# snap-research/R2L

Hardware: AMD Instinct MI355X
Metric: rays/sec (train+render) W256D88 lego@400x400 (higher is better)
Workload: dtype f32 (v_mfma_f32_32x32x2_f32: exact fp32 products and accumulate)

## Files before the change

### r2l_amd/csrc/r2l_dw.h

```cpp
#pragma once
#include "r2l_student_net.h"

#define DW_CHUNK 64
#ifndef DW_DEPTH
#define DW_DEPTH 4
#endif
#ifndef DW_LONG_TRIP
#define DW_LONG_TRIP 128
#endif

struct R2LDwArgs {
    const float* save_x;
    const float* save_t;
    const float* gx;
    const float* gt;
    float* grads;
    int n_block;
    int layer0;
    int n_layers;
    int64_t N;
    int64_t units_per_layer;
    int64_t units_per_wg;
    float* slab;
    float unscale = 1.0f;
    const float* scale_dev = nullptr;
    unsigned* status = nullptr;
    const unsigned* run_if = nullptr;
    unsigned mid_off = 0u;
    const float* act_scale = nullptr;
};

#define DW_SLAB_FLOATS (R2L_W * R2L_W + R2L_W)
#define DW_MAX_WGS 256
#define DW_HEAD_SLAB_MAX ((int64_t)64 * R2L_W * 1024)
#define DW_BODY_SLAB ((int64_t)DW_MAX_WGS * 2 * DW_SLAB_FLOATS)
#define DW_TAIL_SLAB_BASE (DW_BODY_SLAB + DW_HEAD_SLAB_MAX)
#define DW_TAIL_SLAB ((int64_t)512 * 4 * R2L_W)

struct R2LDwHeadArgs {
    const float* rays_o;
    const float* rays_d;
    const float* t_rand;
    const float* ztab;
    const float* emb;
    const float* gh;
    float* slab;
    float* grads;
    int64_t N;
    int64_t rays_per_wg;
    float gscale = 1.0f, unscale = 1.0f;
    const float* scale_dev = nullptr;
    const unsigned* run_unless = nullptr;
    const unsigned* run_if = nullptr;
    bool exact = false;
};

struct PECol {
    int smp, ax;
    float scale;
    int kind;
};
__device__ __forceinline__ PECol pe_col(int k) {
    PECol c;
    if (k >= R2L_IN) { c.smp = 0; c.ax = 0; c.scale = 0.f; c.kind = 3; return c; }
    const int co = k / 21, f = k - 21 * co;
    c.smp = co / 3;
    c.ax = co - 3 * c.smp;
    c.kind = f == 20 ? 2 : (f < 10 ? 0 : 1);
    c.scale = f == 20 ? 1.f : (float)(1 << (f < 10 ? f : f - 10));
    return c;
}
__device__ __forceinline__ float pe_eval(const PECol& c, float x) {
    float s, co;
    r2l_sincos(x * c.scale, s, co);
    const float t = c.kind == 0 ? s : co;
    return c.kind == 2 ? x : (c.kind == 3 ? 0.f : t);
}

int r2l_dw_head16_launch(const R2LDwHeadArgs& a, int64_t slices, hipStream_t stream);

int r2l_dw16_launch(const R2LDwArgs& a, int64_t wgs, const unsigned* run_unless, hipStream_t stream);

int r2l_bwd2_open_step(unsigned* status, const float* params, int n_block, float grad_scale, const float* drgb, int64_t N,
                       hipStream_t stream);
int r2l_dw_body_launch(R2LDwArgs a, int dw_body, int64_t wgs, unsigned* status, bool no_fallback, hipStream_t stream);
int r2l_dw_head_launch(R2LDwHeadArgs a, int64_t slices, bool dw_head16, const unsigned* status, bool no_fallback,
                       hipStream_t stream);
int r2l_dw_tail_launch(const float* dpre, const float* x0, const float* xn, float* grads, float* part, int n_block, int64_t N,
                       int64_t wgs, int64_t rays_per_wg, hipStream_t stream);
```

### r2l_amd/csrc/r2l_dw_head.hip

```cpp
#include "r2l_dw.h"

struct HeadStep {
    f32x4 g0, g1;
    float o0, d0, u0, o1, d1, u1;
};

template <bool FROM_EMB, bool JITTER>
__global__ __launch_bounds__(256, 1) void r2l_dw_head_kernel(const R2LDwHeadArgs a) {
    if (a.run_if != nullptr && __builtin_nontemporal_load(a.run_if) == 0u) return;
    const int wave = threadIdx.x >> 6, lane = threadIdx.x & 63;
    const int hh = lane >> 5, jl = lane & 31;
    const int kq = blockIdx.x & 3;
    const int64_t slice = blockIdx.x >> 2;
    const int64_t r0 = slice * a.rays_per_wg;
    int64_t r1 = r0 + a.rays_per_wg;
    if (r1 > a.N) r1 = a.N;
    if (r0 >= r1) return;
    const int kbase = kq * 256 + wave * 64;
    constexpr bool from_emb = FROM_EMB;
    constexpr bool jitter = JITTER && !FROM_EMB;
    const int k0 = kbase + jl, k1 = kbase + 32 + jl;
    const PECol c0 = pe_col(k0), c1 = pe_col(k1);
    const int e0 = k0 < R2L_IN ? k0 : R2L_IN - 1, e1 = k1 < R2L_IN ? k1 : R2L_IN - 1;
    const float m0 = k0 < R2L_IN ? 1.f : 0.f, m1 = k1 < R2L_IN ? 1.f : 0.f;
    const float zl0 = from_emb ? 0.f : a.ztab[c0.smp], zs0 = jitter ? a.ztab[16 + c0.smp] : 0.f;
    const float zl1 = from_emb ? 0.f : a.ztab[c1.smp], zs1 = jitter ? a.ztab[16 + c1.smp] : 0.f;

    f32x16 acc[8][2];
#pragma unroll
    for (int eo = 0; eo < 8; ++eo)
#pragma unroll
        for (int ei = 0; ei < 2; ++ei)
#pragma unroll
            for (int c = 0; c < 16; ++c) acc[eo][ei][c] = 0.f;
    f32x4 bs0 = {0.f, 0.f, 0.f, 0.f}, bs1 = {0.f, 0.f, 0.f, 0.f};

    const int64_t nfull = (r1 - r0) / 2;
    auto ld = [&](int64_t s, HeadStep& v) {
        const int64_t sc = s < nfull ? s : (nfull > 0 ? nfull - 1 : 0);
        const int64_t r = r0 + 2 * sc + hh;
        v.g0 = *reinterpret_cast<const f32x4*>(a.gh + r * R2L_W + 4 * jl);
        v.g1 = *reinterpret_cast<const f32x4*>(a.gh + r * R2L_W + 128 + 4 * jl);
        if constexpr (from_emb) {
            v.o0 = a.emb[r * R2L_IN + e0];
            v.o1 = a.emb[r * R2L_IN + e1];
            v.d0 = v.d1 = v.u0 = v.u1 = 0.f;
        } else {
            v.o0 = a.rays_o[r * 3 + c0.ax]; v.d0 = a.rays_d[r * 3 + c0.ax];
            v.o1 = a.rays_o[r * 3 + c1.ax]; v.d1 = a.rays_d[r * 3 + c1.ax];
            if constexpr (jitter) {
                v.u0 = a.t_rand[r * 16 + c0.smp];
                v.u1 = a.t_rand[r * 16 + c1.smp];
            } else {
                v.u0 = v.u1 = 0.f;
            }
        }
    };
    auto encode = [&](const HeadStep& v, float& p0, float& p1) {
        if constexpr (from_emb) { p0 = v.o0 * m0; p1 = v.o1 * m1; return; }
        const float z0 = jitter ? zl0 + zs0 * v.u0 : zl0;
        const float z1 = jitter ? zl1 + zs1 * v.u1 : zl1;
        p0 = pe_eval(c0, v.o0 + v.d0 * z0);
        p1 = pe_eval(c1, v.o1 + v.d1 * z1);
    };
    auto kstep = [&](const f32x4& g0, const f32x4& g1, float p0, float p1) {
#pragma unroll
        for (int e = 0; e < 4; ++e) {
            acc[e][0] = __builtin_amdgcn_mfma_f32_32x32x2f32(g0[e], p0, acc[e][0], 0, 0, 0);
            acc[e][1] = __builtin_amdgcn_mfma_f32_32x32x2f32(g0[e], p1, acc[e][1], 0, 0, 0);
            acc[4 + e][0] = __builtin_amdgcn_mfma_f32_32x32x2f32(g1[e], p0, acc[4 + e][0], 0, 0, 0);
            acc[4 + e][1] = __builtin_amdgcn_mfma_f32_32x32x2f32(g1[e], p1, acc[4 + e][1], 0, 0, 0);
        }
        bs0 += g0;
        bs1 += g1;
    };
    if (nfull > 0) {
        HeadStep hb[4];
#pragma unroll
        for (int k = 0; k < 4; ++k) ld(k, hb[k]);
        float pa0, pa1;
        encode(hb[0], pa0, pa1);
        int64_t s = 0;
        for (; s + 16 <= nfull; s += 16) {
#pragma unroll
            for (int k = 0; k < 16; ++k) {
                const f32x4 g0 = hb[k & 3].g0, g1 = hb[k & 3].g1;
                float pn0, pn1;
                encode(hb[(k + 1) & 3], pn0, pn1);
                kstep(g0, g1, pa0, pa1);
                ld(s + k + 4, hb[k & 3]);
                pa0 = pn0;
                pa1 = pn1;
                __builtin_amdgcn_sched_barrier(0);
            }
        }
        for (; s < nfull; ++s) {
            HeadStep v;
            ld(s, v);
            float p0, p1;
            encode(v, p0, p1);
            kstep(v.g0, v.g1, p0, p1);
        }
    }
    if ((r1 - r0) & 1) {
        const int64_t r = r1 - 1;
        HeadStep v;
        v.g0 = *reinterpret_cast<const f32x4*>(a.gh + r * R2L_W + 4 * jl);
        v.g1 = *reinterpret_cast<const f32x4*>(a.gh + r * R2L_W + 128 + 4 * jl);
        if constexpr (from_emb) {
            v.o0 = a.emb[r * R2L_IN + e0];
            v.o1 = a.emb[r * R2L_IN + e1];
            v.d0 = v.d1 = v.u0 = v.u1 = 0.f;
        } else {
            v.o0 = a.rays_o[r * 3 + c0.ax]; v.d0 = a.rays_d[r * 3 + c0.ax];
            v.o1 = a.rays_o[r * 3 + c1.ax]; v.d1 = a.rays_d[r * 3 + c1.ax];
            v.u0 = jitter ? a.t_rand[r * 16 + c0.smp] : 0.f;
            v.u1 = jitter ? a.t_rand[r * 16 + c1.smp] : 0.f;
        }
        float p0, p1;
        encode(v, p0, p1);
        if (hh) { v.g0 = f32x4{0.f, 0.f, 0.f, 0.f}; v.g1 = v.g0; p0 = 0.f; p1 = 0.f; }
        kstep(v.g0, v.g1, p0, p1);
    }
    float* gw = a.grads;
    float* sl = a.slab ? a.slab + slice * (int64_t)(R2L_W * 1024) : nullptr;
#pragma unroll
    for (int eo = 0; eo < 8; ++eo)
#pragma unroll
        for (int ei = 0; ei < 2; ++ei)
#pragma unroll
            for (int c = 0; c < 16; ++c) {
                const int ro = (c & 3) + 8 * (c >> 2) + 4 * hh;
                const int o = (eo >> 2) * 128 + 4 * ro + (eo & 3);
                const int k = kbase + ei * 32 + jl;
                if (k < R2L_IN) {
                    if (sl) sl[o * 1024 + k] = acc[eo][ei][c];
                    else atomicAdd(gw + (int64_t)o * R2L_IN + k, acc[eo][ei][c]);
                }
            }
    if (kq == 0 && wave == 0) {
        float* gb = a.grads + r2l_off_head_b();
#pragma unroll
        for (int e = 0; e < 4; ++e) {
            const float s0 = bs0[e] + __shfl_xor(bs0[e], 32);
            const float s1 = bs1[e] + __shfl_xor(bs1[e], 32);
            if (hh == 0) {
                if (sl) {
                    sl[(4 * jl + e) * 1024 + R2L_IN] = s0;
                    sl[(128 + 4 * jl + e) * 1024 + R2L_IN] = s1;
                } else {
                    atomicAdd(gb + 4 * jl + e, s0);
                    atomicAdd(gb + 128 + 4 * jl + e, s1);
                }
            }
        }
    }
}

__global__ void r2l_head_reduce_kernel(const float* __restrict__ slab, int n_slices, float* __restrict__ grads) {
    const int64_t i = (int64_t)blockIdx.x * blockDim.x + threadIdx.x;
    if (i >= (int64_t)R2L_W * 1024) return;
    const int o = (int)(i >> 10), k = (int)(i & 1023);
    if (k > R2L_IN) return;
    float s = 0.f;
    for (int sidx = 0; sidx < n_slices; ++sidx) s += slab[(int64_t)sidx * (R2L_W * 1024) + i];
    if (k == R2L_IN) grads[r2l_off_head_b() + o] += s;
    else grads[(int64_t)o * R2L_IN + k] += s;
}

int r2l_dw_head_launch(R2LDwHeadArgs a, int64_t slices, bool dw_head16, const unsigned* status, bool no_fallback,
                       hipStream_t stream) {
    const dim3 hg((unsigned)(slices * 4)), hb(256);
    if (dw_head16) {
        a.run_unless = status;
        if (const int rc = r2l_dw_head16_launch(a, slices, stream)) return rc;
        a.run_unless = nullptr;
        a.run_if = status;
    }
    if (dw_head16 && no_fallback) {
    } else if (a.emb != nullptr) hipLaunchKernelGGL((r2l_dw_head_kernel<true, false>), hg, hb, 0, stream, a);
    else if (a.t_rand != nullptr) hipLaunchKernelGGL((r2l_dw_head_kernel<false, true>), hg, hb, 0, stream, a);
    else hipLaunchKernelGGL((r2l_dw_head_kernel<false, false>), hg, hb, 0, stream, a);
    R2L_CHECK(hipGetLastError());
    if (a.slab) {
        hipLaunchKernelGGL(r2l_head_reduce_kernel, dim3(R2L_W * 1024 / 256), dim3(256), 0, stream, a.slab, (int)slices, a.grads);
        R2L_CHECK(hipGetLastError());
    }
    return 0;
}
```

### r2l_amd/csrc/r2l_dw_head16.hip

```cpp
#include "r2l_f2.h"
#include "r2l_dw.h"

struct Head16G {
    float g[8][8];
};
struct Head16Rays {
    float oa[8], da[8], ua[8], ob[8], db[8], ub[8];
};
struct Head16Pair {
    int ka, kb;
    int smp_a, ax_a;
    int smp_b, ax_b;
    float scale;
    bool trig;
};
__device__ __forceinline__ Head16Pair head16_pair(int P) {
    Head16Pair c;
    if (P < 480) {
        const int co = P / 10, f = P - 10 * co;
        c.ka = 21 * co + f; c.kb = 21 * co + 10 + f;
        c.smp_a = c.smp_b = co / 3; c.ax_a = c.ax_b = co % 3;
        c.scale = (float)(1 << f); c.trig = true;
    } else {
        const int i = P - 480, ca = 2 * i, cb = 2 * i + 1;
        const bool live = i < 24;
        c.ka = live ? 21 * ca + 20 : -1; c.kb = live ? 21 * cb + 20 : -1;
        c.smp_a = live ? ca / 3 : 0; c.ax_a = live ? ca % 3 : 0;
        c.smp_b = live ? cb / 3 : 0; c.ax_b = live ? cb % 3 : 0;
        c.scale = 1.f; c.trig = false;
    }
    return c;
}

typedef __amdgpu_buffer_rsrc_t h16_rsrc_t;
__device__ __forceinline__ float h16_load(h16_rsrc_t rs, unsigned voff, unsigned imm) {
    return __builtin_bit_cast(float, __builtin_amdgcn_raw_buffer_load_b32(rs, voff + imm, 0, 0));
}
__device__ __forceinline__ h16_rsrc_t h16_rsrc(const float* base, unsigned bytes) {
    return __builtin_amdgcn_make_buffer_rsrc(const_cast<float*>(base), 0, (int)bytes, 0x00020000);
}

template <bool JITTER, bool EXACT>
__global__ __launch_bounds__(256, 1) void r2l_dw_head16_kernel(const R2LDwHeadArgs a) {
    if (a.run_unless != nullptr && __builtin_nontemporal_load(a.run_unless) != 0u) return;
    const float gscale = a.scale_dev != nullptr ? a.scale_dev[0] : a.gscale;
    const float unscale = a.scale_dev != nullptr ? a.scale_dev[1] : a.unscale;
    const int lane = threadIdx.x & 63;
    const int wave = __builtin_amdgcn_readfirstlane((int)(threadIdx.x >> 6));
    const int m = lane & 31, kg = lane >> 5;
    const int kq = blockIdx.x & 3;
    const int64_t slice = blockIdx.x >> 2;
    const int64_t r0 = slice * a.rays_per_wg;
    int64_t r1 = r0 + a.rays_per_wg;
    if (r1 > a.N) r1 = a.N;
    if (r0 >= r1) return;
    const int nrays = (int)(r1 - r0);
    const Head16Pair pc = head16_pair(kq * 128 + wave * 32 + m);
    const bool trig_wave = kq * 128 + wave * 32 + 31 < 480;
    const float zla = a.ztab[pc.smp_a], zsa = JITTER ? a.ztab[16 + pc.smp_a] : 0.f;
    const float zlb = a.ztab[pc.smp_b], zsb = JITTER ? a.ztab[16 + pc.smp_b] : 0.f;

    f32x16 acc[8][2];
#pragma unroll
    for (int e = 0; e < 8; ++e)
#pragma unroll
        for (int ei = 0; ei < 2; ++ei)
#pragma unroll
            for (int c = 0; c < 16; ++c) acc[e][ei][c] = 0.f;
    float bsum[8] = {0.f, 0.f, 0.f, 0.f, 0.f, 0.f, 0.f, 0.f};

    const h16_rsrc_t grs = h16_rsrc(a.gh + r0 * R2L_W, (unsigned)nrays * (R2L_W * 4));
    const h16_rsrc_t ors = h16_rsrc(a.rays_o + r0 * 3, (unsigned)nrays * 12u);
    const h16_rsrc_t drs = h16_rsrc(a.rays_d + r0 * 3, (unsigned)nrays * 12u);
    const h16_rsrc_t urs = h16_rsrc(JITTER ? a.t_rand + r0 * 16 : a.rays_o, JITTER ? (unsigned)nrays * 64u : 0u);
    unsigned vg = (unsigned)((8 * kg * R2L_W + m) * 4);
    unsigned vp0 = (unsigned)((8 * kg * 3 + pc.ax_a) * 4), vp1 = (unsigned)((8 * kg * 3 + pc.ax_b) * 4);
    unsigned vu0 = (unsigned)((8 * kg * 16 + pc.smp_a) * 4), vu1 = (unsigned)((8 * kg * 16 + pc.smp_b) * 4);
    const int nsteps = (nrays + 15) / 16;

    auto ld_g = [&](Head16G& v) {
#pragma unroll
        for (int i = 0; i < 8; ++i)
#pragma unroll
            for (int e = 0; e < 8; ++e)
                v.g[e][i] = (i < 4) ? h16_load(grs, vg, (unsigned)(i * 1024 + e * 128))
                                    : h16_load(grs, vg + 4096u, (unsigned)((i - 4) * 1024 + e * 128));
        vg += 16u * R2L_W * 4u;
    };
    auto ld_rays = [&](Head16Rays& v) {
#pragma unroll
        for (int i = 0; i < 8; ++i) {
            v.oa[i] = h16_load(ors, vp0, (unsigned)i * 12u);
            v.da[i] = h16_load(drs, vp0, (unsigned)i * 12u);
            v.ua[i] = JITTER ? h16_load(urs, vu0, (unsigned)i * 64u) : 0.f;
            if (!trig_wave) {
                v.ob[i] = h16_load(ors, vp1, (unsigned)i * 12u);
                v.db[i] = h16_load(drs, vp1, (unsigned)i * 12u);
                v.ub[i] = JITTER ? h16_load(urs, vu1, (unsigned)i * 64u) : 0.f;
            } else {
                v.ob[i] = v.db[i] = v.ub[i] = 0.f;
            }
        }
        vp0 += 16u * 12u; vp1 += 16u * 12u;
        vu0 += 16u * 64u; vu1 += 16u * 64u;
    };
    auto pk = [](float x0, float x1) { return F2Side<false, F3None>::pk(x0, x1); };
    Head16G rg;
    Head16Rays rr;
    ld_g(rg);
    ld_rays(rr);
    for (int s = 0; s < nsteps; ++s) {
        f16x8 ga[8], gm[EXACT ? 8 : 1];
        const float sc = gscale;
#pragma unroll
        for (int e = 0; e < 8; ++e) {
            u32x4 uh;
#pragma unroll
            for (int d = 0; d < 4; ++d) uh[d] = pk(rg.g[e][2 * d] * sc, rg.g[e][2 * d + 1] * sc);
            ga[e] = __builtin_bit_cast(f16x8, uh);
            if (EXACT) {
                u32x4 um;
#pragma unroll
                for (int d = 0; d < 4; ++d)
                    um[d] = pk(f2_res_lo(uh[d], rg.g[e][2 * d] * sc), f2_res_hi(uh[d], rg.g[e][2 * d + 1] * sc));
                gm[e] = __builtin_bit_cast(f16x8, um);
            }
            if (kq == 0 && wave == 0)
                bsum[e] += ((rg.g[e][0] + rg.g[e][1]) + (rg.g[e][2] + rg.g[e][3])) + ((rg.g[e][4] + rg.g[e][5]) + (rg.g[e][6] + rg.g[e][7]));
        }
        __builtin_amdgcn_sched_barrier(0);
        ld_g(rg);
        __builtin_amdgcn_sched_barrier(0);
        float p0[8], p1[8];
#pragma unroll
        for (int i = 0; i < 8; ++i) {
            const float xa = rr.oa[i] + rr.da[i] * (JITTER ? zla + zsa * rr.ua[i] : zla);
            if (trig_wave) {
                r2l_sincos(xa * pc.scale, p0[i], p1[i]);
            } else {
                const float xb = rr.ob[i] + rr.db[i] * (JITTER ? zlb + zsb * rr.ub[i] : zlb);
                float sn, cs;
                r2l_sincos(xa * pc.scale, sn, cs);
                p0[i] = pc.trig ? sn : (pc.ka >= 0 ? xa : 0.f);
                p1[i] = pc.trig ? cs : (pc.kb >= 0 ? xb : 0.f);
            }
        }
        u32x4 u0, u1, m0, m1;
#pragma unroll
        for (int d = 0; d < 4; ++d) {
            u0[d] = pk(p0[2 * d], p0[2 * d + 1]);
            u1[d] = pk(p1[2 * d], p1[2 * d + 1]);
            if (EXACT) {
                m0[d] = pk(f2_res_lo(u0[d], p0[2 * d]), f2_res_hi(u0[d], p0[2 * d + 1]));
                m1[d] = pk(f2_res_lo(u1[d], p1[2 * d]), f2_res_hi(u1[d], p1[2 * d + 1]));
            }
        }
        const f16x8 b0 = __builtin_bit_cast(f16x8, u0), b1 = __builtin_bit_cast(f16x8, u1);
        __builtin_amdgcn_sched_barrier(0);
        ld_rays(rr);
        __builtin_amdgcn_sched_barrier(0);
        if (EXACT) {
            const f16x8 bm0 = __builtin_bit_cast(f16x8, m0), bm1 = __builtin_bit_cast(f16x8, m1);
#pragma unroll
            for (int e = 0; e < 8; ++e) {
                acc[e][0] = __builtin_amdgcn_mfma_f32_32x32x16_f16(gm[e], b0, acc[e][0], 0, 0, 0);
                acc[e][1] = __builtin_amdgcn_mfma_f32_32x32x16_f16(gm[e], b1, acc[e][1], 0, 0, 0);
            }
#pragma unroll
            for (int e = 0; e < 8; ++e) {
                acc[e][0] = __builtin_amdgcn_mfma_f32_32x32x16_f16(ga[e], bm0, acc[e][0], 0, 0, 0);
                acc[e][1] = __builtin_amdgcn_mfma_f32_32x32x16_f16(ga[e], bm1, acc[e][1], 0, 0, 0);
            }
        }
#pragma unroll
        for (int e = 0; e < 8; ++e) {
            acc[e][0] = __builtin_amdgcn_mfma_f32_32x32x16_f16(ga[e], b0, acc[e][0], 0, 0, 0);
            acc[e][1] = __builtin_amdgcn_mfma_f32_32x32x16_f16(ga[e], b1, acc[e][1], 0, 0, 0);
        }
    }
    float* sl = a.slab ? a.slab + slice * (int64_t)(R2L_W * 1024) : nullptr;
#pragma unroll
    for (int ei = 0; ei < 2; ++ei) {
        const int k = ei == 0 ? pc.ka : pc.kb;
        if (k < 0) continue;
        if (sl) {
            float* p = sl + (4 * kg) * 1024 + k;
#pragma unroll
            for (int e = 0; e < 8; ++e)
#pragma unroll
                for (int c = 0; c < 16; ++c) p[(32 * e + 8 * (c >> 2) + (c & 3)) * 1024] = acc[e][ei][c] * unscale;
        } else {
            float* p = a.grads + (int64_t)(4 * kg) * R2L_IN + k;
#pragma unroll
            for (int e = 0; e < 8; ++e)
#pragma unroll
                for (int c = 0; c < 16; ++c) atomicAdd(p + (32 * e + 8 * (c >> 2) + (c & 3)) * R2L_IN, acc[e][ei][c] * unscale);
        }
    }
    if (kq == 0 && wave == 0) {
#pragma unroll
        for (int e = 0; e < 8; ++e) {
            const float s = bsum[e] + __shfl_xor(bsum[e], 32);
            if (kg == 0) {
                if (sl) sl[(32 * e + m) * 1024 + R2L_IN] = s;
                else atomicAdd(a.grads + r2l_off_head_b() + 32 * e + m, s);
            }
        }
    }
}

int r2l_dw_head16_launch(const R2LDwHeadArgs& a, int64_t slices, hipStream_t stream) {
    const dim3 grid((unsigned)(slices * 4)), block(256);
    if (a.exact) {
        if (a.t_rand != nullptr) hipLaunchKernelGGL((r2l_dw_head16_kernel<true, true>), grid, block, 0, stream, a);
        else hipLaunchKernelGGL((r2l_dw_head16_kernel<false, true>), grid, block, 0, stream, a);
    } else {
        if (a.t_rand != nullptr) hipLaunchKernelGGL((r2l_dw_head16_kernel<true, false>), grid, block, 0, stream, a);
        else hipLaunchKernelGGL((r2l_dw_head16_kernel<false, false>), grid, block, 0, stream, a);
    }
    R2L_CHECK(hipGetLastError());
    return 0;
}
```

Before: 12.60 million.

## Stage head dW gradients through double-buffered LDS and pair trig columns

The fp16 head dW kernel now loads each gradient row once per workgroup, converts it to f16 (with residuals in exact mode) a single time, and stages it through a double-buffered LDS image. Previously every wave converted its own copy. Ray origin, direction and jitter values are staged the same way, and the bias sums are spread across waves and then reduced through LDS. The fp32 head kernel is changed to pair sin and cos columns so one sincos serves two outputs, and it uses buffer loads with incrementing offsets and an MFMA interleave schedule. The head-reduce kernel batches 16 slab loads at a time. In exchange, the kernels add per-step workgroup barriers and LDS traffic.

Measured after the change: 12.62 million (median of 3 runs). Within noise of the previous version (+0.1%).

```diff
diff --git a/r2l_amd/csrc/r2l_dw.h b/r2l_amd/csrc/r2l_dw.h
--- a/r2l_amd/csrc/r2l_dw.h
+++ b/r2l_amd/csrc/r2l_dw.h
@@ -55,26 +55,29 @@
     bool exact = false;
 };
 
-struct PECol {
-    int smp, ax;
+struct Head16Pair {
+    int ka, kb;
+    int smp_a, ax_a;
+    int smp_b, ax_b;
     float scale;
-    int kind;
+    bool trig;
 };
-__device__ __forceinline__ PECol pe_col(int k) {
-    PECol c;
-    if (k >= R2L_IN) { c.smp = 0; c.ax = 0; c.scale = 0.f; c.kind = 3; return c; }
-    const int co = k / 21, f = k - 21 * co;
-    c.smp = co / 3;
-    c.ax = co - 3 * c.smp;
-    c.kind = f == 20 ? 2 : (f < 10 ? 0 : 1);
-    c.scale = f == 20 ? 1.f : (float)(1 << (f < 10 ? f : f - 10));
+__device__ __forceinline__ Head16Pair head16_pair(int P) {
+    Head16Pair c;
+    if (P < 480) {
+        const int co = P / 10, f = P - 10 * co;
+        c.ka = 21 * co + f; c.kb = 21 * co + 10 + f;
+        c.smp_a = c.smp_b = co / 3; c.ax_a = c.ax_b = co % 3;
+        c.scale = (float)(1 << f); c.trig = true;
+    } else {
+        const int i = P - 480, ca = 2 * i, cb = 2 * i + 1;
+        const bool live = i < 24;
+        c.ka = live ? 21 * ca + 20 : -1; c.kb = live ? 21 * cb + 20 : -1;
+        c.smp_a = live ? ca / 3 : 0; c.ax_a = live ? ca % 3 : 0;
+        c.smp_b = live ? cb / 3 : 0; c.ax_b = live ? cb % 3 : 0;
+        c.scale = 1.f; c.trig = false;
+    }
     return c;
-}
-__device__ __forceinline__ float pe_eval(const PECol& c, float x) {
-    float s, co;
-    r2l_sincos(x * c.scale, s, co);
-    const float t = c.kind == 0 ? s : co;
-    return c.kind == 2 ? x : (c.kind == 3 ? 0.f : t);
 }
 
 int r2l_dw_head16_launch(const R2LDwHeadArgs& a, int64_t slices, hipStream_t stream);
diff --git a/r2l_amd/csrc/r2l_dw_head.hip b/r2l_amd/csrc/r2l_dw_head.hip
--- a/r2l_amd/csrc/r2l_dw_head.hip
+++ b/r2l_amd/csrc/r2l_dw_head.hip
@@ -1,3 +1,4 @@
+#include <type_traits>
 #include "r2l_dw.h"
 
 struct HeadStep {
@@ -5,10 +6,21 @@
     float o0, d0, u0, o1, d1, u1;
 };
 
+typedef __amdgpu_buffer_rsrc_t head_rsrc_t;
+__device__ __forceinline__ head_rsrc_t head_rsrc(const float* base, unsigned bytes) {
+    return __builtin_amdgcn_make_buffer_rsrc(const_cast<float*>(base), 0, (int)bytes, 0x00020000);
+}
+__device__ __forceinline__ float head_load(head_rsrc_t rs, unsigned voff) {
+    return __builtin_bit_cast(float, __builtin_amdgcn_raw_buffer_load_b32(rs, voff, 0, 0));
+}
+__device__ __forceinline__ f32x4 head_load4(head_rsrc_t rs, unsigned voff) {
+    return __builtin_bit_cast(f32x4, __builtin_amdgcn_raw_buffer_load_b128(rs, voff, 0, 0));
+}
+
 template <bool FROM_EMB, bool JITTER>
 __global__ __launch_bounds__(256, 1) void r2l_dw_head_kernel(const R2LDwHeadArgs a) {
     if (a.run_if != nullptr && __builtin_nontemporal_load(a.run_if) == 0u) return;
-    const int wave = threadIdx.x >> 6, lane = threadIdx.x & 63;
+    const int wave = __builtin_amdgcn_readfirstlane((int)(threadIdx.x >> 6)), lane = threadIdx.x & 63;
     const int hh = lane >> 5, jl = lane & 31;
     const int kq = blockIdx.x & 3;
     const int64_t slice = blockIdx.x >> 2;
@@ -16,15 +28,15 @@
     int64_t r1 = r0 + a.rays_per_wg;
     if (r1 > a.N) r1 = a.N;
     if (r0 >= r1) return;
-    const int kbase = kq * 256 + wave * 64;
+    const int nrays = (int)(r1 - r0);
     constexpr bool from_emb = FROM_EMB;
     constexpr bool jitter = JITTER && !FROM_EMB;
-    const int k0 = kbase + jl, k1 = kbase + 32 + jl;
-    const PECol c0 = pe_col(k0), c1 = pe_col(k1);
-    const int e0 = k0 < R2L_IN ? k0 : R2L_IN - 1, e1 = k1 < R2L_IN ? k1 : R2L_IN - 1;
-    const float m0 = k0 < R2L_IN ? 1.f : 0.f, m1 = k1 < R2L_IN ? 1.f : 0.f;
-    const float zl0 = from_emb ? 0.f : a.ztab[c0.smp], zs0 = jitter ? a.ztab[16 + c0.smp] : 0.f;
-    const float zl1 = from_emb ? 0.f : a.ztab[c1.smp], zs1 = jitter ? a.ztab[16 + c1.smp] : 0.f;
+    const Head16Pair pc = head16_pair(kq * 128 + wave * 32 + jl);
+    const bool trig_wave = kq * 128 + wave * 32 + 31 < 480;
+    const int e0 = pc.ka >= 0 ? pc.ka : 0, e1 = pc.kb >= 0 ? pc.kb : 0;
+    const float m0 = pc.ka >= 0 ? 1.f : 0.f, m1 = pc.kb >= 0 ? 1.f : 0.f;
+    const float zl0 = from_emb ? 0.f : a.ztab[pc.smp_a], zs0 = jitter ? a.ztab[16 + pc.smp_a] : 0.f;
+    const float zl1 = from_emb ? 0.f : a.ztab[pc.smp_b], zs1 = jitter ? a.ztab[16 + pc.smp_b] : 0.f;
 
     f32x16 acc[8][2];
 #pragma unroll
@@ -35,35 +47,48 @@
             for (int c = 0; c < 16; ++c) acc[eo][ei][c] = 0.f;
     f32x4 bs0 = {0.f, 0.f, 0.f, 0.f}, bs1 = {0.f, 0.f, 0.f, 0.f};
 
-    const int64_t nfull = (r1 - r0) / 2;
-    auto ld = [&](int64_t s, HeadStep& v) {
-        const int64_t sc = s < nfull ? s : (nfull > 0 ? nfull - 1 : 0);
-        const int64_t r = r0 + 2 * sc + hh;
-        v.g0 = *reinterpret_cast<const f32x4*>(a.gh + r * R2L_W + 4 * jl);
-        v.g1 = *reinterpret_cast<const f32x4*>(a.gh + r * R2L_W + 128 + 4 * jl);
-        if constexpr (from_emb) {
-            v.o0 = a.emb[r * R2L_IN + e0];
-            v.o1 = a.emb[r * R2L_IN + e1];
-            v.d0 = v.d1 = v.u0 = v.u1 = 0.f;
-        } else {
-            v.o0 = a.rays_o[r * 3 + c0.ax]; v.d0 = a.rays_d[r * 3 + c0.ax];
-            v.o1 = a.rays_o[r * 3 + c1.ax]; v.d1 = a.rays_d[r * 3 + c1.ax];
-            if constexpr (jitter) {
-                v.u0 = a.t_rand[r * 16 + c0.smp];
-                v.u1 = a.t_rand[r * 16 + c1.smp];
-            } else {
-                v.u0 = v.u1 = 0.f;
-            }
-        }
-    };
-    auto encode = [&](const HeadStep& v, float& p0, float& p1) {
-        if constexpr (from_emb) { p0 = v.o0 * m0; p1 = v.o1 * m1; return; }
-        const float z0 = jitter ? zl0 + zs0 * v.u0 : zl0;
-        const float z1 = jitter ? zl1 + zs1 * v.u1 : zl1;
-        p0 = pe_eval(c0, v.o0 + v.d0 * z0);
-        p1 = pe_eval(c1, v.o1 + v.d1 * z1);
-    };
-    auto kstep = [&](const f32x4& g0, const f32x4& g1, float p0, float p1) {
+    const head_rsrc_t grs = head_rsrc(a.gh + r0 * R2L_W, (unsigned)nrays * (R2L_W * 4));
+    const head_rsrc_t ors = head_rsrc(from_emb ? a.emb + r0 * R2L_IN : a.rays_o + r0 * 3, (unsigned)nrays * (from_emb ? R2L_IN * 4u : 12u));
+    const head_rsrc_t drs = head_rsrc(from_emb ? a.gh : a.rays_d + r0 * 3, from_emb ? 0u : (unsigned)nrays * 12u);
+    const head_rsrc_t urs = head_rsrc(jitter ? a.t_rand + r0 * 16 : a.gh, jitter ? (unsigned)nrays * 64u : 0u);
+    unsigned vg = (unsigned)(hh * (R2L_W * 4) + jl * 16);
+    unsigned vp0 = from_emb ? (unsigned)((hh * R2L_IN + e0) * 4) : (unsigned)((hh * 3 + pc.ax_a) * 4);
+    unsigned vp1 = from_emb ? (unsigned)((hh * R2L_IN + e1) * 4) : (unsigned)((hh * 3 + pc.ax_b) * 4);
+    unsigned vu0 = (unsigned)((hh * 16 + pc.smp_a) * 4), vu1 = (unsigned)((hh * 16 + pc.smp_b) * 4);
+    const int nsteps = (nrays + 1) / 2;
+
+    auto ld = [&](auto trig, HeadStep& v) __attribute__((always_inline)) {
+        constexpr bool TRIG = decltype(trig)::value;
+        v.g0 = head_load4(grs, vg);
+        v.g1 = head_load4(grs, vg + 512u);
+        vg += 2u * R2L_W * 4u;
+        v.d0 = v.d1 = v.u0 = v.u1 = v.o1 = 0.f;
+        v.o0 = head_load(ors, vp0);
+        if (from_emb || !TRIG) v.o1 = head_load(ors, vp1);
+        vp0 += from_emb ? 2u * R2L_IN * 4u : 24u;
+        vp1 += from_emb ? 2u * R2L_IN * 4u : 24u;
+        if (!from_emb) {
+            v.d0 = head_load(drs, vp0 - 24u);
+            if (!TRIG) v.d1 = head_load(drs, vp1 - 24u);
+            if (jitter) {
+                v.u0 = head_load(urs, vu0);
+                if (!TRIG) v.u1 = head_load(urs, vu1);
+                vu0 += 128u; vu1 += 128u;
+            }
+        }
+    };
+    auto encode = [&](auto trig, const HeadStep& v, float& p0, float& p1) __attribute__((always_inline)) {
+        constexpr bool TRIG = decltype(trig)::value;
+        if (from_emb) { p0 = v.o0 * m0; p1 = v.o1 * m1; return; }
+        const float xa = v.o0 + v.d0 * (jitter ? zl0 + zs0 * v.u0 : zl0);
+        float sn, cs;
+        r2l_sincos(xa * pc.scale, sn, cs);
+        if (TRIG) { p0 = sn; p1 = cs; return; }
+        const float xb = v.o1 + v.d1 * (jitter ? zl1 + zs1 * v.u1 : zl1);
+        p0 = pc.trig ? sn : (pc.ka >= 0 ? xa : 0.f);
+        p1 = pc.trig ? cs : (pc.kb >= 0 ? xb : 0.f);
+    };
+    auto kstep = [&](const f32x4& g0, const f32x4& g1, float p0, float p1) __attribute__((always_inline)) {
 #pragma unroll
         for (int e = 0; e < 4; ++e) {
             acc[e][0] = __builtin_amdgcn_mfma_f32_32x32x2f32(g0[e], p0, acc[e][0], 0, 0, 0);
@@ -74,54 +99,58 @@
         bs0 += g0;
         bs1 += g1;
     };
-    if (nfull > 0) {
+    auto run = [&](auto trig) __attribute__((always_inline)) {
         HeadStep hb[4];
 #pragma unroll
-        for (int k = 0; k < 4; ++k) ld(k, hb[k]);
+        for (int k = 0; k < 4; ++k) ld(trig, hb[k]);
         float pa0, pa1;
-        encode(hb[0], pa0, pa1);
-        int64_t s = 0;
-        for (; s + 16 <= nfull; s += 16) {
+        encode(trig, hb[0], pa0, pa1);
+        int s = 0;
+        for (; s + 16 <= nsteps; s += 16) {
 #pragma unroll
             for (int k = 0; k < 16; ++k) {
                 const f32x4 g0 = hb[k & 3].g0, g1 = hb[k & 3].g1;
                 float pn0, pn1;
-                encode(hb[(k + 1) & 3], pn0, pn1);
+                encode(trig, hb[(k + 1) & 3], pn0, pn1);
                 kstep(g0, g1, pa0, pa1);
-                ld(s + k + 4, hb[k & 3]);
+                ld(trig, hb[k & 3]);
+                pa0 = pn0;
+                pa1 = pn1;
+#pragma unroll
+                for (int i = 0; i < 16; ++i) {
+                    __builtin_amdgcn_sched_group_barrier(0x008, 1, 0);
+                    __builtin_amdgcn_sched_group_barrier(0x002, 4, 0);
+                    if (i < 8) __builtin_amdgcn_sched_group_barrier(0x020, 1, 0);
+                }
+                __builtin_amdgcn_sched_barrier(0);
+            }
+        }
+        for (; s + 4 <= nsteps; s += 4) {
+#pragma unroll
+            for (int k = 0; k < 4; ++k) {
+                const f32x4 g0 = hb[k].g0, g1 = hb[k].g1;
+                float pn0, pn1;
+                encode(trig, hb[(k + 1) & 3], pn0, pn1);
+                kstep(g0, g1, pa0, pa1);
+                ld(trig, hb[k]);
                 pa0 = pn0;
                 pa1 = pn1;
                 __builtin_amdgcn_sched_barrier(0);
             }
         }
-        for (; s < nfull; ++s) {
-            HeadStep v;
-            ld(s, v);
-            float p0, p1;
-            encode(v, p0, p1);
-            kstep(v.g0, v.g1, p0, p1);
-        }
-    }
-    if ((r1 - r0) & 1) {
-        const int64_t r = r1 - 1;
-        HeadStep v;
-        v.g0 = *reinterpret_cast<const f32x4*>(a.gh + r * R2L_W + 4 * jl);
-        v.g1 = *reinterpret_cast<const f32x4*>(a.gh + r * R2L_W + 128 + 4 * jl);
-        if constexpr (from_emb) {
-            v.o0 = a.emb[r * R2L_IN + e0];
-            v.o1 = a.emb[r * R2L_IN + e1];
-            v.d0 = v.d1 = v.u0 = v.u1 = 0.f;
-        } else {
-            v.o0 = a.rays_o[r * 3 + c0.ax]; v.d0 = a.rays_d[r * 3 + c0.ax];
-            v.o1 = a.rays_o[r * 3 + c1.ax]; v.d1 = a.rays_d[r * 3 + c1.ax];
-            v.u0 = jitter ? a.t_rand[r * 16 + c0.smp] : 0.f;
-            v.u1 = jitter ? a.t_rand[r * 16 + c1.smp] : 0.f;
-        }
-        float p0, p1;
-        encode(v, p0, p1);
-        if (hh) { v.g0 = f32x4{0.f, 0.f, 0.f, 0.f}; v.g1 = v.g0; p0 = 0.f; p1 = 0.f; }
-        kstep(v.g0, v.g1, p0, p1);
-    }
+#pragma unroll
+        for (int k = 0; k < 3; ++k) {
+            if (s + k < nsteps) {
+                float pn0, pn1;
+                encode(trig, hb[k + 1], pn0, pn1);
+                kstep(hb[k].g0, hb[k].g1, pa0, pa1);
+                pa0 = pn0;
+                pa1 = pn1;
+            }
+        }
+    };
+    if (trig_wave) run(std::true_type{});
+    else run(std::false_type{});
     float* gw = a.grads;
     float* sl = a.slab ? a.slab + slice * (int64_t)(R2L_W * 1024) : nullptr;
 #pragma unroll
@@ -132,8 +161,8 @@
             for (int c = 0; c < 16; ++c) {
                 const int ro = (c & 3) + 8 * (c >> 2) + 4 * hh;
                 const int o = (eo >> 2) * 128 + 4 * ro + (eo & 3);
-                const int k = kbase + ei * 32 + jl;
-                if (k < R2L_IN) {
+                const int k = ei == 0 ? pc.ka : pc.kb;
+                if (k >= 0) {
                     if (sl) sl[o * 1024 + k] = acc[eo][ei][c];
                     else atomicAdd(gw + (int64_t)o * R2L_IN + k, acc[eo][ei][c]);
                 }
@@ -157,13 +186,23 @@
     }
 }
 
+#define DW_HEAD_REDUCE_AHEAD 16
 __global__ void r2l_head_reduce_kernel(const float* __restrict__ slab, int n_slices, float* __restrict__ grads) {
     const int64_t i = (int64_t)blockIdx.x * blockDim.x + threadIdx.x;
     if (i >= (int64_t)R2L_W * 1024) return;
     const int o = (int)(i >> 10), k = (int)(i & 1023);
     if (k > R2L_IN) return;
     float s = 0.f;
-    for (int sidx = 0; sidx < n_slices; ++sidx) s += slab[(int64_t)sidx * (R2L_W * 1024) + i];
+    const float* p = slab + i;
+    int sidx = 0;
+    for (; sidx + DW_HEAD_REDUCE_AHEAD <= n_slices; sidx += DW_HEAD_REDUCE_AHEAD) {
+        float v[DW_HEAD_REDUCE_AHEAD];
+#pragma unroll
+        for (int j = 0; j < DW_HEAD_REDUCE_AHEAD; ++j) v[j] = p[(int64_t)(sidx + j) * (R2L_W * 1024)];
+#pragma unroll
+        for (int j = 0; j < DW_HEAD_REDUCE_AHEAD; ++j) s += v[j];
+    }
+    for (; sidx < n_slices; ++sidx) s += p[(int64_t)sidx * (R2L_W * 1024)];
     if (k == R2L_IN) grads[r2l_off_head_b() + o] += s;
     else grads[(int64_t)o * R2L_IN + k] += s;
 }
diff --git a/r2l_amd/csrc/r2l_dw_head16.hip b/r2l_amd/csrc/r2l_dw_head16.hip
--- a/r2l_amd/csrc/r2l_dw_head16.hip
+++ b/r2l_amd/csrc/r2l_dw_head16.hip
@@ -1,47 +1,35 @@
+#include <type_traits>
 #include "r2l_f2.h"
 #include "r2l_dw.h"
 
-struct Head16G {
-    float g[8][8];
+typedef unsigned u32x2 __attribute__((ext_vector_type(2)));
+struct Head16Stage {
+    f32x4 g[4];
+    float od, u;
 };
 struct Head16Rays {
     float oa[8], da[8], ua[8], ob[8], db[8], ub[8];
 };
-struct Head16Pair {
-    int ka, kb;
-    int smp_a, ax_a;
-    int smp_b, ax_b;
-    float scale;
-    bool trig;
-};
-__device__ __forceinline__ Head16Pair head16_pair(int P) {
-    Head16Pair c;
-    if (P < 480) {
-        const int co = P / 10, f = P - 10 * co;
-        c.ka = 21 * co + f; c.kb = 21 * co + 10 + f;
-        c.smp_a = c.smp_b = co / 3; c.ax_a = c.ax_b = co % 3;
-        c.scale = (float)(1 << f); c.trig = true;
-    } else {
-        const int i = P - 480, ca = 2 * i, cb = 2 * i + 1;
-        const bool live = i < 24;
-        c.ka = live ? 21 * ca + 20 : -1; c.kb = live ? 21 * cb + 20 : -1;
-        c.smp_a = live ? ca / 3 : 0; c.ax_a = live ? ca % 3 : 0;
-        c.smp_b = live ? cb / 3 : 0; c.ax_b = live ? cb % 3 : 0;
-        c.scale = 1.f; c.trig = false;
-    }
-    return c;
-}
-
 typedef __amdgpu_buffer_rsrc_t h16_rsrc_t;
 __device__ __forceinline__ float h16_load(h16_rsrc_t rs, unsigned voff, unsigned imm) {
     return __builtin_bit_cast(float, __builtin_amdgcn_raw_buffer_load_b32(rs, voff + imm, 0, 0));
 }
+__device__ __forceinline__ f32x4 h16_load4(h16_rsrc_t rs, unsigned voff, unsigned imm) {
+    return __builtin_bit_cast(f32x4, __builtin_amdgcn_raw_buffer_load_b128(rs, voff + imm, 0, 0));
+}
 __device__ __forceinline__ h16_rsrc_t h16_rsrc(const float* base, unsigned bytes) {
     return __builtin_amdgcn_make_buffer_rsrc(const_cast<float*>(base), 0, (int)bytes, 0x00020000);
 }
 
+#define H16_IMG_BYTES 8192
+#define H16_RAY_BYTES 1536
+__device__ __forceinline__ int h16_chunk(int m, int kg) { return 32 * kg + 8 * (m & 3) + ((m >> 2) ^ ((m & 2) << 1)); }
+
 template <bool JITTER, bool EXACT>
 __global__ __launch_bounds__(256, 1) void r2l_dw_head16_kernel(const R2LDwHeadArgs a) {
+    constexpr int RAY_OFF = H16_IMG_BYTES * (EXACT ? 2 : 1);
+    constexpr int BUF_BYTES = RAY_OFF + H16_RAY_BYTES;
+    __shared__ __attribute__((aligned(16))) unsigned char lds[2 * BUF_BYTES];
     if (a.run_unless != nullptr && __builtin_nontemporal_load(a.run_unless) != 0u) return;
     const float gscale = a.scale_dev != nullptr ? a.scale_dev[0] : a.gscale;
     const float unscale = a.scale_dev != nullptr ? a.scale_dev[1] : a.unscale;
@@ -67,75 +55,93 @@
         for (int ei = 0; ei < 2; ++ei)
 #pragma unroll
             for (int c = 0; c < 16; ++c) acc[e][ei][c] = 0.f;
-    float bsum[8] = {0.f, 0.f, 0.f, 0.f, 0.f, 0.f, 0.f, 0.f};
-
+
+    const int shalf = lane & 1, skg = wave >> 1;
+    const int sj = (lane >> 1) + 32 * (wave & 1), sq = 2 * skg + shalf;
+    float bsum[4] = {0.f, 0.f, 0.f, 0.f};
     const h16_rsrc_t grs = h16_rsrc(a.gh + r0 * R2L_W, (unsigned)nrays * (R2L_W * 4));
-    const h16_rsrc_t ors = h16_rsrc(a.rays_o + r0 * 3, (unsigned)nrays * 12u);
-    const h16_rsrc_t drs = h16_rsrc(a.rays_d + r0 * 3, (unsigned)nrays * 12u);
+    const h16_rsrc_t odrs = h16_rsrc(((wave & 1) == 0 ? a.rays_o : a.rays_d) + r0 * 3, (unsigned)nrays * 12u);
     const h16_rsrc_t urs = h16_rsrc(JITTER ? a.t_rand + r0 * 16 : a.rays_o, JITTER ? (unsigned)nrays * 64u : 0u);
-    unsigned vg = (unsigned)((8 * kg * R2L_W + m) * 4);
-    unsigned vp0 = (unsigned)((8 * kg * 3 + pc.ax_a) * 4), vp1 = (unsigned)((8 * kg * 3 + pc.ax_b) * 4);
-    unsigned vu0 = (unsigned)((8 * kg * 16 + pc.smp_a) * 4), vu1 = (unsigned)((8 * kg * 16 + pc.smp_b) * 4);
+    unsigned vg = (unsigned)(4 * sq * (R2L_W * 4) + sj * 16);
+    unsigned vu = (unsigned)(((threadIdx.x & 15) * 16 + (threadIdx.x >> 4)) * 4);
+    unsigned vod = (unsigned)(((lane & 15) * 3 + ((lane >> 4) < 2 ? (lane >> 4) : 2)) * 4);
     const int nsteps = (nrays + 15) / 16;
-
-    auto ld_g = [&](Head16G& v) {
-#pragma unroll
-        for (int i = 0; i < 8; ++i)
-#pragma unroll
-            for (int e = 0; e < 8; ++e)
-                v.g[e][i] = (i < 4) ? h16_load(grs, vg, (unsigned)(i * 1024 + e * 128))
-                                    : h16_load(grs, vg + 4096u, (unsigned)((i - 4) * 1024 + e * 128));
+    const unsigned wr_a = (unsigned)((64 * (sj >> 3) + 32 * skg + (sj & 7)) * 16 + 8 * shalf);
+    const unsigned wr_b = (unsigned)((64 * (sj >> 3) + 32 * skg + ((sj & 7) ^ 4)) * 16 + 8 * shalf);
+    const unsigned wr_u = (unsigned)(RAY_OFF + (128 + threadIdx.x) * 4), wr_od = (unsigned)(RAY_OFF + (64 * (wave & 1) + lane) * 4);
+    const unsigned rd_g = (unsigned)(h16_chunk(m, kg) * 16);
+    const unsigned rd_pa = (unsigned)(RAY_OFF + (16 * pc.ax_a + 8 * kg) * 4), rd_pb = (unsigned)(RAY_OFF + (16 * pc.ax_b + 8 * kg) * 4);
+    const unsigned rd_ua = (unsigned)(RAY_OFF + (128 + 16 * pc.smp_a + 8 * kg) * 4);
+    const unsigned rd_ub = (unsigned)(RAY_OFF + (128 + 16 * pc.smp_b + 8 * kg) * 4);
+
+    auto ld = [&](Head16Stage& v) {
+#pragma unroll
+        for (int i = 0; i < 4; ++i) v.g[i] = h16_load4(grs, vg, (unsigned)(i * R2L_W * 4));
         vg += 16u * R2L_W * 4u;
-    };
-    auto ld_rays = [&](Head16Rays& v) {
-#pragma unroll
-        for (int i = 0; i < 8; ++i) {
-            v.oa[i] = h16_load(ors, vp0, (unsigned)i * 12u);
-            v.da[i] = h16_load(drs, vp0, (unsigned)i * 12u);
-            v.ua[i] = JITTER ? h16_load(urs, vu0, (unsigned)i * 64u) : 0.f;
-            if (!trig_wave) {
-                v.ob[i] = h16_load(ors, vp1, (unsigned)i * 12u);
-                v.db[i] = h16_load(drs, vp1, (unsigned)i * 12u);
-                v.ub[i] = JITTER ? h16_load(urs, vu1, (unsigned)i * 64u) : 0.f;
-            } else {
-                v.ob[i] = v.db[i] = v.ub[i] = 0.f;
-            }
-        }
-        vp0 += 16u * 12u; vp1 += 16u * 12u;
-        vu0 += 16u * 64u; vu1 += 16u * 64u;
+        v.u = 0.f;
+        if (JITTER) { v.u = h16_load(urs, vu, 0u); vu += 16u * 64u; }
+        v.od = h16_load(odrs, vod, 0u);
+        vod += 16u * 12u;
     };
     auto pk = [](float x0, float x1) { return F2Side<false, F3None>::pk(x0, x1); };
-    Head16G rg;
-    Head16Rays rr;
-    ld_g(rg);
-    ld_rays(rr);
-    for (int s = 0; s < nsteps; ++s) {
+    auto stage = [&](const Head16Stage& v, unsigned buf) {
+        unsigned char* b = lds + buf;
+#pragma unroll
+        for (int cc = 0; cc < 4; ++cc) {
+            float x[4];
+#pragma unroll
+            for (int i = 0; i < 4; ++i) x[i] = v.g[i][cc];
+            u32x2 uh;
+            uh[0] = pk(x[0] * gscale, x[1] * gscale);
+            uh[1] = pk(x[2] * gscale, x[3] * gscale);
+            const unsigned off = (cc < 2 ? wr_a : wr_b) + 128u * cc;
+            *reinterpret_cast<u32x2*>(b + off) = uh;
+            if (EXACT) {
+                u32x2 um;
+                um[0] = pk(f2_res_lo(uh[0], x[0] * gscale), f2_res_hi(uh[0], x[1] * gscale));
+                um[1] = pk(f2_res_lo(uh[1], x[2] * gscale), f2_res_hi(uh[1], x[3] * gscale));
+                *reinterpret_cast<u32x2*>(b + H16_IMG_BYTES + off) = um;
+            }
+            float q01 = x[0] + x[1], q23 = x[2] + x[3];
+            r2l_no_pack(q01);
+            r2l_no_pack(q23);
+            const float q4 = q01 + q23;
+            const float o4 = __builtin_bit_cast(float, __builtin_amdgcn_update_dpp(0, __builtin_bit_cast(int, q4), 0xB1, 0xF, 0xF, false));
+            bsum[cc] += q4 + o4;
+        }
+        if (JITTER) *reinterpret_cast<float*>(b + wr_u) = v.u;
+        *reinterpret_cast<float*>(b + wr_od) = v.od;
+    };
+    auto rd8 = [&](const unsigned char* b, unsigned off, float (&out)[8]) {
+        const f32x4 lo = *reinterpret_cast<const f32x4*>(b + off), hi = *reinterpret_cast<const f32x4*>(b + off + 16);
+#pragma unroll
+        for (int i = 0; i < 4; ++i) { out[i] = lo[i]; out[4 + i] = hi[i]; }
+    };
+    auto kstep = [&](auto trig, Head16Stage& nx, unsigned rb) __attribute__((always_inline)) {
+        constexpr bool TRIG = decltype(trig)::value;
+        const unsigned char* b = lds + rb;
+        Head16Rays rr;
+        rd8(b, rd_pa, rr.oa);
+        rd8(b, rd_pa + 256u, rr.da);
+#pragma unroll
+        for (int i = 0; i < 8; ++i) rr.ua[i] = rr.ob[i] = rr.db[i] = rr.ub[i] = 0.f;
+        if (JITTER) rd8(b, rd_ua, rr.ua);
+        if (!TRIG) {
+            rd8(b, rd_pb, rr.ob);
+            rd8(b, rd_pb + 256u, rr.db);
+            if (JITTER) rd8(b, rd_ub, rr.ub);
+        }
         f16x8 ga[8], gm[EXACT ? 8 : 1];
-        const float sc = gscale;
 #pragma unroll
         for (int e = 0; e < 8; ++e) {
-            u32x4 uh;
-#pragma unroll
-            for (int d = 0; d < 4; ++d) uh[d] = pk(rg.g[e][2 * d] * sc, rg.g[e][2 * d + 1] * sc);
-            ga[e] = __builtin_bit_cast(f16x8, uh);
-            if (EXACT) {
-                u32x4 um;
-#pragma unroll
-                for (int d = 0; d < 4; ++d)
-                    um[d] = pk(f2_res_lo(uh[d], rg.g[e][2 * d] * sc), f2_res_hi(uh[d], rg.g[e][2 * d + 1] * sc));
-                gm[e] = __builtin_bit_cast(f16x8, um);
-            }
-            if (kq == 0 && wave == 0)
-                bsum[e] += ((rg.g[e][0] + rg.g[e][1]) + (rg.g[e][2] + rg.g[e][3])) + ((rg.g[e][4] + rg.g[e][5]) + (rg.g[e][6] + rg.g[e][7]));
-        }
-        __builtin_amdgcn_sched_barrier(0);
-        ld_g(rg);
-        __builtin_amdgcn_sched_barrier(0);
+            ga[e] = *reinterpret_cast<const f16x8*>(b + rd_g + 1024u * e);
+            if (EXACT) gm[e] = *reinterpret_cast<const f16x8*>(b + H16_IMG_BYTES + rd_g + 1024u * e);
+        }
         float p0[8], p1[8];
 #pragma unroll
         for (int i = 0; i < 8; ++i) {
             const float xa = rr.oa[i] + rr.da[i] * (JITTER ? zla + zsa * rr.ua[i] : zla);
-            if (trig_wave) {
+            if (TRIG) {
                 r2l_sincos(xa * pc.scale, p0[i], p1[i]);
             } else {
                 const float xb = rr.ob[i] + rr.db[i] * (JITTER ? zlb + zsb * rr.ub[i] : zlb);
@@ -157,7 +163,9 @@
         }
         const f16x8 b0 = __builtin_bit_cast(f16x8, u0), b1 = __builtin_bit_cast(f16x8, u1);
         __builtin_amdgcn_sched_barrier(0);
-        ld_rays(rr);
+        stage(nx, (unsigned)BUF_BYTES - rb);
+        __builtin_amdgcn_sched_barrier(0);
+        ld(nx);
         __builtin_amdgcn_sched_barrier(0);
         if (EXACT) {
             const f16x8 bm0 = __builtin_bit_cast(f16x8, m0), bm1 = __builtin_bit_cast(f16x8, m1);
@@ -177,7 +185,46 @@
             acc[e][0] = __builtin_amdgcn_mfma_f32_32x32x16_f16(ga[e], b0, acc[e][0], 0, 0, 0);
             acc[e][1] = __builtin_amdgcn_mfma_f32_32x32x16_f16(ga[e], b1, acc[e][1], 0, 0, 0);
         }
-    }
+        __builtin_amdgcn_fence(__ATOMIC_RELEASE, "workgroup", "local");
+        __builtin_amdgcn_s_barrier();
+        __builtin_amdgcn_fence(__ATOMIC_ACQUIRE, "workgroup", "local");
+    };
+
+    Head16Stage s0, s1, s2, s3;
+    ld(s0);
+    ld(s1);
+    ld(s2);
+    ld(s3);
+    stage(s0, 0u);
+    ld(s0);
+    __builtin_amdgcn_fence(__ATOMIC_RELEASE, "workgroup", "local");
+    __builtin_amdgcn_s_barrier();
+    __builtin_amdgcn_fence(__ATOMIC_ACQUIRE, "workgroup", "local");
+    auto run = [&](auto trig) __attribute__((always_inline)) {
+        int s = 0;
+        for (; s + 8 <= nsteps; s += 8) {
+            kstep(trig, s1, 0u);
+            kstep(trig, s2, (unsigned)BUF_BYTES);
+            kstep(trig, s3, 0u);
+            kstep(trig, s0, (unsigned)BUF_BYTES);
+            kstep(trig, s1, 0u);
+            kstep(trig, s2, (unsigned)BUF_BYTES);
+            kstep(trig, s3, 0u);
+            kstep(trig, s0, (unsigned)BUF_BYTES);
+        }
+        if (s + 4 <= nsteps) {
+            kstep(trig, s1, 0u);
+            kstep(trig, s2, (unsigned)BUF_BYTES);
+            kstep(trig, s3, 0u);
+            kstep(trig, s0, (unsigned)BUF_BYTES);
+            s += 4;
+        }
+        if (s < nsteps) kstep(trig, s1, 0u);
+        if (s + 1 < nsteps) kstep(trig, s2, (unsigned)BUF_BYTES);
+        if (s + 2 < nsteps) kstep(trig, s3, 0u);
+    };
+    if (trig_wave) run(std::true_type{});
+    else run(std::false_type{});
     float* sl = a.slab ? a.slab + slice * (int64_t)(R2L_W * 1024) : nullptr;
 #pragma unroll
     for (int ei = 0; ei < 2; ++ei) {
@@ -197,13 +244,20 @@
                 for (int c = 0; c < 16; ++c) atomicAdd(p + (32 * e + 8 * (c >> 2) + (c & 3)) * R2L_IN, acc[e][ei][c] * unscale);
         }
     }
-    if (kq == 0 && wave == 0) {
-#pragma unroll
-        for (int e = 0; e < 8; ++e) {
-            const float s = bsum[e] + __shfl_xor(bsum[e], 32);
-            if (kg == 0) {
-                if (sl) sl[(32 * e + m) * 1024 + R2L_IN] = s;
-                else atomicAdd(a.grads + r2l_off_head_b() + 32 * e + m, s);
+    if (kq == 0) {
+        float* xch = reinterpret_cast<float*>(lds);
+        if (skg == 1 && shalf == 0) {
+#pragma unroll
+            for (int cc = 0; cc < 4; ++cc) xch[4 * sj + cc] = bsum[cc];
+        }
+        __syncthreads();
+        if (skg == 0 && shalf == 0) {
+#pragma unroll
+            for (int cc = 0; cc < 4; ++cc) {
+                const int o = 4 * sj + cc;
+                const float s = bsum[cc] + xch[o];
+                if (sl) sl[o * 1024 + R2L_IN] = s;
+                else atomicAdd(a.grads + r2l_off_head_b() + o, s);
             }
         }
     }
```
